# OllieBoyne/sslap

Hardware: AMD Instinct MI355X
Metric: Medges/s (bid-phase CSR nnz/s) + solve ms, N=200k d=0.1% sparse LAP (higher is better)
Workload: dtype f64

## Files before the change

### sslap_amd/csrc/device_common.hpp

```cpp
#pragma once
#include <hip/hip_runtime.h>
#include <stdint.h>

#include <type_traits>

namespace misslap {

constexpr int kWave = 64;
constexpr int kPosNone = 0x7fffffff;
constexpr int kTailMax = 512;

#define MISSLAP_KERNEL(BLOCK) MISSLAP_KERNEL_BOUND(BLOCK, BLOCK)
#define MISSLAP_KERNEL_BOUND(BLOCK, BOUND)                                                          \
    static constexpr int kBlock = (BLOCK);    \
    static constexpr int kBound = (BOUND);      \
    static_assert(kBlock <= kBound, "a launch above the kernel's bound fails");                     \
    template <class... A_>                                                                          \
    static __global__ __launch_bounds__(BOUND) void entry(A_... a_) {                               \
        run(a_...);                                                                                 \
    }

constexpr int kErrNegativeBid = 1;
constexpr int kErrRowsUnsorted = 2;
constexpr int kErrRowGap = 4;
// ... 105 lines not shown
}

__device__ __forceinline__ bool dense_entry_valid(double v) {
    const unsigned long long b = (unsigned long long)__double_as_longlong(v);
    return b <= 0x7ff0000000000000ull || b == 0x8000000000000000ull;
}
__device__ __forceinline__ bool bid_is_bad(double bid) {
    const unsigned long long b = (unsigned long long)__double_as_longlong(bid);
    return b > 0x7ff0000000000000ull;
}

__device__ __forceinline__ double shfl_xor_f64(double v, int off) {
    int lo = __double2loint(v), hi = __double2hiint(v);
    lo = __shfl_xor(lo, off);
    hi = __shfl_xor(hi, off);
    return __hiloint2double(hi, lo);
}

struct NoStamp {
    __device__ __forceinline__ void operator()(int) const {}
    __device__ __forceinline__ void light(int) const {}
};
struct CycleStamp {
    unsigned long long *acc;
    unsigned long long *prev;
    bool on;
    __device__ __forceinline__ void operator()(int k) const {
        asm volatile("s_waitcnt vmcnt(0) lgkmcnt(0)" ::: "memory");
        const unsigned long long t = __builtin_amdgcn_s_memtime();
        if (on) acc[k] += t - *prev;
        *prev = t;
    }
    __device__ __forceinline__ void light(int k) const {
        const unsigned long long t = __builtin_amdgcn_s_memtime();
        if (on) acc[k] += t - *prev;
        *prev = t;
    }
};

constexpr int kDppXor1 = 0xB1;
constexpr int kDppXor2 = 0x4E;
constexpr int kDppHalfMirror = 0x141;
constexpr int kDppMirror = 0x140;
constexpr int kDppBcast15 = 0x142;
constexpr int kDppBcast31 = 0x143;
template <int CTRL, int ROW_MASK = 0xF>
__device__ __forceinline__ int dpp_i32(int v) {
    return __builtin_amdgcn_update_dpp(v, v, CTRL, ROW_MASK, 0xF, false);
}
template <int CTRL, int ROW_MASK = 0xF>
__device__ __forceinline__ double dpp_f64(double v) {
    const int lo = dpp_i32<CTRL, ROW_MASK>(__double2loint(v));
    const int hi = dpp_i32<CTRL, ROW_MASK>(__double2hiint(v));
    return __hiloint2double(hi, lo);
}
__device__ __forceinline__ double readlane_f64(double v, int l) {
    const int lo = __builtin_amdgcn_readlane(__double2loint(v), l);
    const int hi = __builtin_amdgcn_readlane(__double2hiint(v), l);
    return __hiloint2double(hi, lo);
}

#define MISSLAP_WAVE_MAX_STEP(T, EXCH) \
    {                                  \
        const T o = EXCH;              \
        v = o > v ? o : v;             \
    }
__device__ __forceinline__ int wave_max_i32(int v) {
    MISSLAP_WAVE_MAX_STEP(int, __builtin_amdgcn_mov_dpp(v, kDppXor1, 0xF, 0xF, true))
    MISSLAP_WAVE_MAX_STEP(int, __builtin_amdgcn_mov_dpp(v, kDppXor2, 0xF, 0xF, true))
    MISSLAP_WAVE_MAX_STEP(int, __builtin_amdgcn_mov_dpp(v, kDppHalfMirror, 0xF, 0xF, true))
    MISSLAP_WAVE_MAX_STEP(int, __builtin_amdgcn_mov_dpp(v, kDppMirror, 0xF, 0xF, true))
    MISSLAP_WAVE_MAX_STEP(int, (dpp_i32<kDppBcast15, 0xA>(v)))
    MISSLAP_WAVE_MAX_STEP(int, (dpp_i32<kDppBcast31, 0xC>(v)))
    return __builtin_amdgcn_readlane(v, 63);
}
__device__ __forceinline__ double wave_max_f64(double v) {
    v = __builtin_fmax(v, dpp_f64<kDppXor1>(v));
    v = __builtin_fmax(v, dpp_f64<kDppXor2>(v));
    v = __builtin_fmax(v, dpp_f64<kDppHalfMirror>(v));
    v = __builtin_fmax(v, dpp_f64<kDppMirror>(v));
    v = __builtin_fmax(v, (dpp_f64<kDppBcast15, 0xA>(v)));
    v = __builtin_fmax(v, (dpp_f64<kDppBcast31, 0xC>(v)));
    return readlane_f64(v, 63);
}
#undef MISSLAP_WAVE_MAX_STEP

struct Top2 {
    double v, w;
    int g;
};
__device__ __forceinline__ Top2 top2_wave_reduce(const Top2 &x) {
    Top2 r;
    r.v = wave_max_f64(x.v);
    r.g = wave_max_i32(x.v == r.v ? x.g : -1);
    r.w = wave_max_f64(x.g == r.g ? x.w : x.v);
    return r;
}

struct __attribute__((aligned(16))) PriceRec {
    double price;
    int owner;
    int ostart;
};

__device__ __forceinline__ int lane_id() { return threadIdx.x & (kWave - 1); }
__device__ __forceinline__ unsigned long long lanemask_lt() {
    return (1ull << lane_id()) - 1ull;
}

constexpr int kCandLanes = 32;
constexpr int kCandMax = 30;
constexpr int kCandMin = 24;
constexpr int kCandRowMax = 4 * kWave;

template <int CTRL>
__device__ __forceinline__ int dppf_i32(int v) {
    return __builtin_amdgcn_mov_dpp(v, CTRL, 0xF, 0xF, true);
}
template <int CTRL>
__device__ __forceinline__ double dppf_f64(double v) {
    return __hiloint2double(dppf_i32<CTRL>(__double2hiint(v)), dppf_i32<CTRL>(__double2loint(v)));
}
__device__ __forceinline__ double half_max_f64(double v) {
    v = __builtin_fmax(v, dppf_f64<kDppXor1>(v));
    v = __builtin_fmax(v, dppf_f64<kDppXor2>(v));
    v = __builtin_fmax(v, dppf_f64<kDppHalfMirror>(v));
    v = __builtin_fmax(v, dppf_f64<kDppMirror>(v));
    v = __builtin_fmax(v, (dpp_f64<kDppBcast15, 0xA>(v)));
    return v;
}
__device__ __forceinline__ int half_max_i32(int v) {
    v = max(v, dppf_i32<kDppXor1>(v));
    v = max(v, dppf_i32<kDppXor2>(v));
    v = max(v, dppf_i32<kDppHalfMirror>(v));
    v = max(v, dppf_i32<kDppMirror>(v));
    v = max(v, (dpp_i32<kDppBcast15, 0xA>(v)));
    return v;
}
__device__ __forceinline__ int half_allmax_i32(int v) {
    v = max(v, dppf_i32<kDppXor1>(v));
    v = max(v, dppf_i32<kDppXor2>(v));
    v = max(v, dppf_i32<kDppHalfMirror>(v));
    v = max(v, dppf_i32<kDppMirror>(v));
    const auto s = __builtin_amdgcn_permlane16_swap(v, v, false, false);
    return max((int)s[0], (int)s[1]);
}

__device__ __forceinline__ double slot_cost(const int2 &s) { return (double)__int_as_float(s.y); }
__device__ __forceinline__ double slot_cost(const Slot64 &s) { return s.c; }
__device__ __forceinline__ double slot_cost_at(const int2 &s, int sl) {
    return (double)__int_as_float(__builtin_amdgcn_readlane(s.y, sl));
}
__device__ __forceinline__ double slot_cost_at(const Slot64 &s, int sl) { return readlane_f64(s.c, sl); }
template <class Slot>
struct LineIO;
template <>
struct LineIO<int2> {
    static __device__ __forceinline__ int2 load(const int2 *cand, const double *, size_t idx) { return cand[idx]; }
    static __device__ __forceinline__ int2 make(int x, int y) { return make_int2(x, y); }
};
template <>
struct LineIO<Slot64> {
    static __device__ __forceinline__ Slot64 load(const int2 *cand, const double *cost, size_t idx) {
        const int2 s = cand[idx];
        Slot64 r;
        r.x = s.x;
        r.y = s.y;
        r.c = cost[idx];
        return r;
    }
    static __device__ __forceinline__ Slot64 make(int x, int y) {
        Slot64 r;
        r.x = x;
        r.y = y;
        r.c = 0.0;
        return r;
    }
};

struct CandBid {
    bool hit;
    unsigned long long key;
    int obj;
    int prev, pstart;
    int len;
};

struct RecSource {
    const PriceRec *rec;
    __device__ __forceinline__ PriceRec get(int col) const { return rec[col]; }
};
struct PriceSource {
    const double *price;
    __device__ __forceinline__ PriceRec get(int col) const {
        PriceRec r;
        r.price = price[col];
        r.owner = -1;
        r.ostart = 0;
        return r;
    }
};

template <class Slot, class Src>
__device__ __forceinline__ PriceRec cand_gather2(const Slot slot, const bool act0, const bool act1, const Src &src) {
    const int lane = lane_id(), l32 = lane & (kCandLanes - 1);
    const bool active = lane < kCandLanes ? act0 : act1;
    const bool is_cand = active & (l32 >= 1) & (l32 <= kCandMax) & (slot.x >= 0);
    return src.get(is_cand ? slot.x : 0);
}
template <class Slot, class Early, class S = NoStamp>
__device__ __forceinline__ void cand_eval2_r(Slot &slot, const PriceRec r, const bool act0, const bool act1,
                                             const double eps, CandBid (&out)[2], int &err, Early &&early,
                                             const S &stamp = S(), int *alive = nullptr);
template <class Slot, class Src, class Early, class S = NoStamp>
__device__ __forceinline__ void cand_eval2(Slot &slot, const bool act0, const bool act1, const Src &src,
                                           const double eps, CandBid (&out)[2], int &err, Early &&early,
                                           const S &stamp = S(), int *alive = nullptr) {
    stamp(1);
    const PriceRec r = cand_gather2(slot, act0, act1, src);
    stamp(2);
    cand_eval2_r(slot, r, act0, act1, eps, out, err, early, stamp, alive);
}
template <class Slot, class Early, class S>
__device__ __forceinline__ void cand_eval2_r(Slot &slot, const PriceRec r, const bool act0, const bool act1,
                                             const double eps, CandBid (&out)[2], int &err, Early &&early,
                                             const S &stamp, int *alive) {
    const int lane = lane_id(), l32 = lane & (kCandLanes - 1);
    const double ninf = -__builtin_huge_val();
    const bool active = lane < kCandLanes ? act0 : act1;
    const bool is_cand = active & (l32 >= 1) & (l32 <= kCandMax) & (slot.x >= 0);
    const double cost = slot_cost(slot);
    double tau[2];
    tau[0] = readlane_f64(__hiloint2double(slot.y, slot.x), 0);
    tau[1] = readlane_f64(__hiloint2double(slot.y, slot.x), kCandLanes);
    out[0].len = __builtin_amdgcn_readlane(slot.x, kCandLanes - 1);
    out[1].len = __builtin_amdgcn_readlane(slot.x, 2 * kCandLanes - 1);
    const double v = is_cand ? cost - r.price : ninf;
    if (alive) {
        const unsigned long long al = __ballot(is_cand & (v >= (lane < kCandLanes ? tau[0] : tau[1])));
        alive[0] = __popc((unsigned)al);
        alive[1] = __popc((unsigned)(al >> 32));
    }
    double V[2], W[2];
    int G[2];
    {
        const double vm = half_max_f64(v);
        V[0] = readlane_f64(vm, 31);
        V[1] = readlane_f64(vm, 63);
        const double Vv = lane < kCandLanes ? V[0] : V[1];
        const int gm = half_max_i32((is_cand & (v == Vv)) ? l32 : -1);
        G[0] = __builtin_amdgcn_readlane(gm, 31);
        G[1] = __builtin_amdgcn_readlane(gm, 63);
    }
    double c1[2];
#pragma unroll
    for (int X = 0; X < 2; ++X) {
        const int sl = kCandLanes * X + max(G[X], 0);
        out[X].obj = __builtin_amdgcn_readlane(slot.x, sl);
        out[X].prev = __builtin_amdgcn_readlane(r.owner, sl);
        out[X].pstart = __builtin_amdgcn_readlane(r.ostart, sl);
        c1[X] = slot_cost_at(slot, sl);
    }
    early(out);
    stamp.light(3);
    const int Gv = lane < kCandLanes ? G[0] : G[1];
    const double wm = half_max_f64(l32 == Gv ? ninf : v);
    W[0] = readlane_f64(wm, 31);
    W[1] = readlane_f64(wm, 63);
#pragma unroll
    for (int X = 0; X < 2; ++X) {
        out[X].hit = (G[X] >= 0) & (V[X] > tau[X]) & (W[X] >= tau[X]);
        const double bid = (c1[X] - W[X]) + eps;
        if (out[X].hit && bid_is_bad(bid)) err |= kErrNegativeBid;
        out[X].key = bid_to_key(bid);
    }
}
template <class Slot, class Src>
__device__ __forceinline__ PriceRec cand_gather1(const Slot &slot, const bool cls, const Src &src) {
    const bool is_cand = cls & (slot.x >= 0);
    return src.get(is_cand ? slot.x : 0);
}
template <class Slot, class Early, class S = NoStamp>
__device__ __forceinline__ void cand_eval1_r(Slot &slot, const PriceRec r, const bool cls, const double eps, CandBid &out,
                                             unsigned &bad_hi, Early &&early, const S &stamp = S());
template <class Slot, class Src, class Early, class S = NoStamp>
__device__ __forceinline__ void cand_eval1(Slot &slot, const bool cls, const Src &src, const double eps, CandBid &out,
                                           unsigned &bad_hi, Early &&early, const S &stamp = S()) {
    stamp(1);
    const PriceRec r = cand_gather1(slot, cls, src);
    stamp(2);
    cand_eval1_r(slot, r, cls, eps, out, bad_hi, early, stamp);
}
template <class Slot, class Early, class S>
__device__ __forceinline__ void cand_eval1_r(Slot &slot, const PriceRec r, const bool cls, const double eps, CandBid &out,
                                             unsigned &bad_hi, Early &&early, const S &stamp) {
    const int lane = lane_id();
    const double ninf = -__builtin_huge_val();
    const bool is_cand = cls & (slot.x >= 0);
    const double cost = slot_cost(slot);
    const double tau = readlane_f64(__hiloint2double(slot.y, slot.x), 0);
    out.len = __builtin_amdgcn_readlane(slot.x, kCandLanes - 1);
    const double v = is_cand ? cost - r.price : ninf;
    const int hi = __double2hiint(v);
    const int k = hi ^ ((hi >> 31) & 0x7fffffff);
    const int km = __builtin_amdgcn_readlane(half_max_i32(k), 31);
    const unsigned eq = (unsigned)(__ballot(k == km) & 0xffffffffull);
    double V;
    int G;
    if (__popc(eq) == 1) {
        G = __ffs((int)eq) - 1;
        V = readlane_f64(v, G);
    } else {
        V = readlane_f64(half_max_f64(v), 31);
        G = __builtin_amdgcn_readlane(half_max_i32((is_cand & (v == V)) ? lane : -1), 31);
    }
    const int sl = max(G, 0);
    out.obj = __builtin_amdgcn_readlane(slot.x, sl);
    out.prev = __builtin_amdgcn_readlane(r.owner, sl);
    out.pstart = __builtin_amdgcn_readlane(r.ostart, sl);
    const double c1 = slot_cost_at(slot, sl);
    early(out);
    stamp.light(3);
    const double W = readlane_f64(half_max_f64(lane == G ? ninf : v), 31);
    out.hit = (G >= 0) & (V > tau) & (W >= tau);
    const double bid = (c1 - W) + eps;
    bad_hi = max(bad_hi, out.hit ? (unsigned)__double2hiint(bid) : 0u);
    out.key = bid_to_key(bid);
}
__device__ __forceinline__ bool bad_hi_is_error(unsigned bad_hi) { return bad_hi > 0x7ff00000u; }
struct NoEarly {
    __device__ __forceinline__ void operator()(const CandBid (&)[2]) const {}
    __device__ __forceinline__ void operator()(const CandBid &) const {}
};

struct CandBuildArgs {
    int c[4];
    double a[4], v[4];
    double V, W;
    int len;
    bool want;
};

__device__ __forceinline__ void cand_build(int2 *cand, double *cost, int person, const CandBuildArgs &ba, double eps,
// ... 266 lines not shown
```

### sslap_amd/csrc/kernels_tail.hpp

```cpp
#pragma once
#include "device_common.hpp"

namespace misslap {

struct TailArgs {
    Ctl *ctl;
    const int *row_ptr;
    double *price;
    PriceRec *rec;
    int *p2o;
    int *o2p;
    int *U;
    int2 *cand;
    double *cand64;
    int thr;
    int round_budget;
    float eps;
};

constexpr int kHashSize = 2048;

__device__ __forceinline__ unsigned long long readlane_u64(unsigned long long v, int l) {
    const int lo = __builtin_amdgcn_readlane((int)(unsigned)(v & 0xffffffffull), l);
    const int hi = __builtin_amdgcn_readlane((int)(unsigned)(v >> 32), l);
    return ((unsigned long long)(unsigned)hi << 32) | (unsigned long long)(unsigned)lo;
}

__device__ __forceinline__ int apply_winner(const TailArgs &a, int person, int pstart, int obj, int prev,
                                            unsigned long long key) {
    PriceRec r;
    r.price = key_to_bid(key);
    r.owner = person;
    r.ostart = pstart;
    a.rec[obj] = r;
    return prev;
}

struct k_sync_from_rec {
    MISSLAP_KERNEL(256)
    static __device__ __forceinline__ void run(Ctl *ctl, const PriceRec *rec, double *price, int *o2p, int *p2o, const int *U, int n_cols, int lines, unsigned long long *live, unsigned ticket) {
        const int K = ctl->K;
        if (blockIdx.x == 0 && threadIdx.x == 0) {
            post_live_status(live, ticket, K, ctl->err, ctl->nits);
            ctl->n_need = 0;
        }
        for (int n = blockIdx.x * blockDim.x + threadIdx.x; n < K; n += gridDim.x * blockDim.x) {
            const int i = U[n];
            if (i >= 0) p2o[i] = -1;
        }
        for (int j = blockIdx.x * blockDim.x + threadIdx.x; j < n_cols; j += gridDim.x * blockDim.x) {
            const PriceRec r = rec[j];
            if (lines && r.price < price[j]) atomicOr(&ctl->err, kErrPriceFell);
            price[j] = r.price;
            o2p[j] = r.owner;
            if (r.owner >= 0) p2o[r.owner] = j;
        }
    }
};


struct TailStats {
    unsigned long long edges, miss_edges, builds;
    unsigned bids, misses;
    unsigned bad_hi;
    int err;
    double hint;
};

__device__ __forceinline__ int lane_zero() {
    return (int)__builtin_amdgcn_mbcnt_hi(0u, __builtin_amdgcn_mbcnt_lo(0u, 0u));
}

template <class Slot>
__device__ __forceinline__ Slot cand_no_line() {
    return (lane_id() & (kCandLanes - 1)) == 0 ? LineIO<Slot>::make(0, 0x7ff00000) : LineIO<Slot>::make(-1, 0);
}
template <class E>
__device__ __forceinline__ typename E::Slot line_of(const TailArgs &a, int p, int l32) {
    return LineIO<typename E::Slot>::load(a.cand, a.cand64, (size_t)max(p, 0) * kCandLanes + l32);
}
template <class E>
struct TwoFetch {
    typename E::Slot slot;
    typename E::Raw row[2][4];
    int ev[2];
};
template <class E>
__device__ __forceinline__ void fetch_row(const TailArgs &a, const E &ed, int person, int start,
                                          typename E::Raw (&row)[4], int &e) {
    const int lane = lane_id();
#pragma unroll
    for (int u = 0; u < 4; ++u) row[u] = ed.load_raw_nt(start + u * kWave + lane);
    e = a.row_ptr[max(person, 0) + 1 + lane_zero()];
}
template <class E>
__device__ __forceinline__ void request_two(const TailArgs &a, const E &ed, int p0, int s0, int p1, int s1,
                                            TwoFetch<E> &tf) {
    if (E::kCand) {
        const int pme = lane_id() < kCandLanes ? p0 : p1;
        tf.slot = a.cand != nullptr ? line_of<E>(a, pme, lane_id() & (kCandLanes - 1)) : cand_no_line<typename E::Slot>();
    } else {
        fetch_row<E>(a, ed, p0, s0, tf.row[0], tf.ev[0]);
        fetch_row<E>(a, ed, p1, s1, tf.row[1], tf.ev[1]);
    }
}

__device__ __forceinline__ void tail_build(const TailArgs &a, int person, const CandBuildArgs &ba, double eps,
                                           TailStats &st) {
    cand_build(a.cand, a.cand64, person, ba, eps, st.hint);
    st.builds += 1;
}

template <class E, class Early, class S = NoStamp>
__device__ __forceinline__ void bid_two(const TailArgs &a, const E &ed, const int (&pi)[2], const int (&ps)[2],
                                        TwoFetch<E> &tf, double eps, CandBid (&b)[2], CandBuildArgs &bd,
                                        int &bd_person, TailStats &st, Early &&early, const S &stamp = S()) {
    const RecSource src{a.rec};
    b[0].hit = b[1].hit = false;
    if (E::kCand) cand_eval2(tf.slot, pi[0] >= 0, pi[1] >= 0, src, eps, b, st.err, early, stamp);
    stamp.light(4);
    bd_person = -1;
#pragma unroll
    for (int X = 0; X < 2; ++X) {
        if (pi[X] < 0) continue;
        if (!b[X].hit) {
            if (bd_person >= 0) tail_build(a, bd_person, bd, eps, st);
            if (E::kCand) {
                const typename E::Raw none[4] = {};
                const int e = a.row_ptr[pi[X] + 1 + lane_zero()];
                wave_bid_full<E, RecSource, true, false>(ed, src, ps[X], e, none, eps, b[X], bd, st.err);
            } else {
                wave_bid_full<E, RecSource, true, true>(ed, src, ps[X], tf.ev[X], tf.row[X], eps, b[X], bd, st.err);
            }
            bd.want = bd.want && a.cand != nullptr;
            bd_person = bd.want ? pi[X] : -1;
            st.misses += 1;
            st.miss_edges += (unsigned long long)b[X].len;
        }
        st.edges += (unsigned long long)b[X].len;
        st.bids += 1;
    }
}

__device__ __forceinline__ int round_limit(long long nits, long long max_iter) {
    return (int)min(max_iter - nits, (long long)0x7fffffff);
}

template <class E>
__device__ __forceinline__ void tail_chain_mode(const TailArgs &a, const E &ed, int &pi, int &ps, int &K,
                                                long long &nits, const long long max_iter, const double eps,
                                                TailStats &st) {
    const int lane = lane_id(), l32 = lane & (kCandLanes - 1);
    const RecSource src{a.rec};
    const bool cls = (lane >= 1) & (lane <= kCandMax);
    const bool lines = E::kCand && a.cand != nullptr;
    typename E::Slot slot = cand_no_line<typename E::Slot>();
    typename E::Raw row[4];
    int ev = 0;
    auto request = [&](int person, int start) {
        if (E::kCand) {
            if (lines) slot = line_of<E>(a, person, l32);
        } else {
            fetch_row<E>(a, ed, person, start, row, ev);
        }
    };
    request(pi, ps);
    const int rmax = round_limit(nits, max_iter);
    int r = 0;
#ifdef MISSLAP_TAIL_STAMP
    unsigned long long sacc[8] = {0, 0, 0, 0, 0, 0, 0, 0}, sprev = __builtin_amdgcn_s_memtime();
    const CycleStamp stamp{sacc, &sprev, true};
#else
    const NoStamp stamp;
#endif
    for (;;) {
        CandBid b;
        b.hit = false;
        int sp = -2;
        if (E::kCand)
            cand_eval1(slot, cls, src, eps, b, st.bad_hi, [&](const CandBid &w) {
                sp = w.prev;
                request(sp, 0);
            }, stamp);
        stamp.light(4);
        if (!b.hit) {
            CandBuildArgs bd;
            if (E::kCand) {
                const typename E::Raw none[4] = {};
                const int e = a.row_ptr[pi + 1];
                wave_bid_full<E, RecSource, true, false>(ed, src, ps, e, none, eps, b, bd, st.err);
            } else {
                wave_bid_full<E, RecSource, true, true>(ed, src, ps, ev, row, eps, b, bd, st.err);
            }
            st.misses += 1;
            st.miss_edges += (unsigned long long)b.len;
            if (bd.want && lines) tail_build(a, pi, bd, eps, st);
        }
        stamp.light(5);
        st.edges += (unsigned long long)b.len;
        st.bids += 1;
        r += 1;
        if (lane == 0) apply_winner(a, pi, ps, b.obj, b.prev, b.key);
        pi = b.prev;
        ps = b.pstart;
        const bool done = pi < 0 || r >= rmax;
        if (!done && sp != pi) request(pi, ps);
        stamp.light(6);
        if (done) break;
    }
    K = pi != -1;
    nits += r;
#ifdef MISSLAP_TAIL_STAMP
    if (lane == 0) {
        for (int k = 1; k <= 6; ++k) a.ctl->dbg[5 + k] += sacc[k];
    }
#endif
}

template <class E>
__device__ __forceinline__ void tail_solo_mode(const TailArgs &a, const E &ed, int *sU, int *sStart, int &K,
                                               long long &nits, const long long max_iter, const double eps,
                                               TailStats &st) {
    const int lane = lane_id();
    int pi[2], ps[2];
    pi[0] = __builtin_amdgcn_readfirstlane(sU[0]);
    ps[0] = __builtin_amdgcn_readfirstlane(sStart[0]);
    pi[1] = K > 1 ? __builtin_amdgcn_readfirstlane(sU[1]) : -1;
    ps[1] = K > 1 ? __builtin_amdgcn_readfirstlane(sStart[1]) : 0;
    if (K == 1) {
        tail_chain_mode(a, ed, pi[0], ps[0], K, nits, max_iter, eps, st);
        if (lane == 0) {
            sU[0] = pi[0];
            sU[1] = -1;
            sStart[0] = ps[0];
        }
        return;
    }
    TwoFetch<E> tf;
    tf.slot = cand_no_line<typename E::Slot>();
    request_two(a, ed, pi[0], ps[0], pi[1], ps[1], tf);
#ifdef MISSLAP_TAIL_STAMP_SOLO
    unsigned long long sacc[8] = {0, 0, 0, 0, 0, 0, 0, 0}, sprev = __builtin_amdgcn_s_memtime();
    const CycleStamp stamp{sacc, &sprev, true};
#else
    const NoStamp stamp;
#endif
    for (;;) {
        CandBid b[2];
        CandBuildArgs bd;
        int bd_person;
        int sp[2] = {-2, -2};
        bid_two(a, ed, pi, ps, tf, eps, b, bd, bd_person, st, [&](const CandBid(&w)[2]) {
            sp[0] = pi[0] >= 0 ? w[0].prev : -1;
            sp[1] = pi[1] >= 0 ? w[1].prev : -1;
            request_two(a, ed, sp[0], 0, sp[1], 0, tf);
        }, stamp);
        stamp.light(5);
        nits += 1;
        bool win0 = true, win1 = pi[1] >= 0;
        if (win1 && b[0].obj == b[1].obj) {
            if (b[1].key > b[0].key) win0 = false;
            else win1 = false;
        }
        if (lane == 0) {
            if (win0) apply_winner(a, pi[0], ps[0], b[0].obj, b[0].prev, b[0].key);
            if (win1) apply_winner(a, pi[1], ps[1], b[1].obj, b[1].prev, b[1].key);
        }
        if (win0) {
            pi[0] = b[0].prev;
            ps[0] = b[0].pstart;
        }
        if (win1) {
            pi[1] = b[1].prev;
            ps[1] = b[1].pstart;
        }
        if (pi[0] == -1 && pi[1] != -1) {
            pi[0] = pi[1];
            ps[0] = ps[1];
            pi[1] = -1;
        }
        K = (pi[0] != -1) + (pi[1] != -1);
        const bool done = K <= 1 || nits >= max_iter;
        if (!done && (sp[0] != pi[0] || sp[1] != pi[1])) request_two(a, ed, pi[0], ps[0], pi[1], ps[1], tf);
        if (bd_person >= 0) tail_build(a, bd_person, bd, eps, st);
        stamp.light(6);
        if (done) break;
    }
    if (K == 1 && nits < max_iter) tail_chain_mode(a, ed, pi[0], ps[0], K, nits, max_iter, eps, st);
#ifdef MISSLAP_TAIL_STAMP_SOLO
    if (lane == 0)
        for (int k = 1; k <= 6; ++k) a.ctl->dbg[5 + k] += sacc[k];
#endif
    if (lane == 0) {
        sU[0] = pi[0];
        sU[1] = pi[1];
        sStart[0] = ps[0];
        sStart[1] = ps[1];
    }
}

template <class E>
__device__ __forceinline__ void tail_pair_mode(const TailArgs &a, const E &ed, int *sU, int *sStart, int &K,
                                               long long &nits, const long long max_iter, const double eps,
                                               TailStats &st) {
    const int lane = lane_id(), l32 = lane & (kCandLanes - 1);
    const bool upper = lane >= kCandLanes;
    const RecSource src{a.rec};
    const bool cls = (l32 >= 1) & (l32 <= kCandMax);
    const double ninf = -__builtin_huge_val();
    int pi[2], ps[2];
#pragma unroll
    for (int X = 0; X < 2; ++X) {
        pi[X] = __builtin_amdgcn_readfirstlane(sU[X]);
        ps[X] = __builtin_amdgcn_readfirstlane(sStart[X]);
    }
    typename E::Slot slot;
    auto request = [&](int p0, int p1) { slot = line_of<E>(a, upper ? p1 : p0, l32); };
    const int rmax = round_limit(nits, max_iter);
    int r = 0;
    if (K == 2) request(pi[0], pi[1]);
#ifdef MISSLAP_TAIL_STAMP_DUO
    unsigned long long sacc[8] = {0, 0, 0, 0, 0, 0, 0, 0}, sprev = __builtin_amdgcn_s_memtime();
    const CycleStamp stamp{sacc, &sprev, true};
#else
    const NoStamp stamp;
#endif
    while (K == 2) {
        stamp(1);
        const PriceRec g = cand_gather1(slot, cls, src);
        stamp(2);
        const bool is_cand = cls & (slot.x >= 0);
        const double v = is_cand ? slot_cost(slot) - g.price : ninf;
        const int hw = __double2hiint(v);
        const int k = hw ^ ((hw >> 31) & 0x7fffffff);
        const unsigned long long eq = __ballot(k == half_allmax_i32(k));
        const unsigned eq0 = (unsigned)eq, eq1 = (unsigned)(eq >> 32);
        int G[2];
        double V[2];
        if ((int)(__popc(eq0) == 1) & (int)(__popc(eq1) == 1)) {
            G[0] = __ffs((int)eq0) - 1;
            G[1] = __ffs((int)eq1) + (kCandLanes - 1);
            V[0] = readlane_f64(v, G[0]);
            V[1] = readlane_f64(v, G[1]);
        } else {
            const double vm = half_max_f64(v);
            V[0] = readlane_f64(vm, kCandLanes - 1);
            V[1] = readlane_f64(vm, kWave - 1);
            const int gm = half_max_i32((is_cand & (v == (upper ? V[1] : V[0]))) ? lane : -1);
            G[0] = __builtin_amdgcn_readlane(gm, kCandLanes - 1);
            G[1] = __builtin_amdgcn_readlane(gm, kWave - 1);
        }
        CandBid b[2];
        double tau[2], c1[2];
#pragma unroll
        for (int X = 0; X < 2; ++X) {
            const int sl = max(G[X], kCandLanes * X);
            tau[X] = readlane_f64(__hiloint2double(slot.y, slot.x), kCandLanes * X);
            b[X].len = __builtin_amdgcn_readlane(slot.x, kCandLanes * X + kCandLanes - 1);
            b[X].obj = __builtin_amdgcn_readlane(slot.x, sl);
            b[X].prev = __builtin_amdgcn_readlane(g.owner, sl);
            b[X].pstart = __builtin_amdgcn_readlane(g.ostart, sl);
            c1[X] = slot_cost_at(slot, sl);
        }
        const int sp0 = b[0].prev, sp1 = b[1].prev;
        request(sp0, sp1);
        stamp.light(3);
        const double wm = half_max_f64(((lane == G[0]) | (lane == G[1])) ? ninf : v);
        const double W[2] = {readlane_f64(wm, kCandLanes - 1), readlane_f64(wm, kWave - 1)};
#pragma unroll
        for (int X = 0; X < 2; ++X) {
            b[X].hit = (G[X] >= 0) & (V[X] > tau[X]) & (W[X] >= tau[X]);
            const double bid = (c1[X] - W[X]) + eps;
            st.bad_hi = max(st.bad_hi, b[X].hit ? (unsigned)__double2hiint(bid) : 0u);
            b[X].key = bid_to_key(bid);
        }
        stamp.light(4);
#pragma unroll
        for (int X = 0; X < 2; ++X) {
            if (!b[X].hit) {
                CandBuildArgs bd;
                const typename E::Raw none[4] = {};
                const int e = a.row_ptr[pi[X] + 1];
                wave_bid_full<E, RecSource, true, false>(ed, src, ps[X], e, none, eps, b[X], bd, st.err);
                st.misses += 1;
                st.miss_edges += (unsigned long long)b[X].len;
                if (bd.want) tail_build(a, pi[X], bd, eps, st);
            }
        }
        stamp.light(5);
        st.edges += (unsigned long long)(b[0].len + b[1].len);
        st.bids += 2;
        r += 1;
        if ((b[0].obj != b[1].obj) & (b[0].prev >= 0) & (b[1].prev >= 0)) {
            if (l32 == 0) {
                PriceRec w;
                w.price = key_to_bid(upper ? b[1].key : b[0].key);
                w.owner = upper ? pi[1] : pi[0];
                w.ostart = upper ? ps[1] : ps[0];
                a.rec[upper ? b[1].obj : b[0].obj] = w;
            }
#pragma unroll
            for (int X = 0; X < 2; ++X) {
                pi[X] = b[X].prev;
                ps[X] = b[X].pstart;
            }
        } else {
            bool win0 = true, win1 = true;
            if (b[0].obj == b[1].obj) {
                if (b[1].key > b[0].key) win0 = false;
                else win1 = false;
            }
            if (lane == 0) {
                if (win0) apply_winner(a, pi[0], ps[0], b[0].obj, b[0].prev, b[0].key);
                if (win1) apply_winner(a, pi[1], ps[1], b[1].obj, b[1].prev, b[1].key);
            }
            if (win0) {
                pi[0] = b[0].prev;
                ps[0] = b[0].pstart;
            }
            if (win1) {
                pi[1] = b[1].prev;
                ps[1] = b[1].pstart;
            }
            if (pi[0] == -1 && pi[1] != -1) {
                pi[0] = pi[1];
                ps[0] = ps[1];
                pi[1] = -1;
            }
            K = (pi[0] != -1) + (pi[1] != -1);
        }
        const bool done = K <= 1 || r >= rmax;
        if (!done && (sp0 != pi[0] || sp1 != pi[1])) request(pi[0], pi[1]);
        stamp.light(6);
        if (done) break;
    }
    nits += r;
#ifdef MISSLAP_TAIL_STAMP_DUO
    if (lane == 0)
        for (int k = 1; k <= 6; ++k) a.ctl->dbg[5 + k] += sacc[k];
#endif
    if (K == 1 && nits < max_iter) tail_chain_mode(a, ed, pi[0], ps[0], K, nits, max_iter, eps, st);
    if (lane == 0) {
        sU[0] = pi[0];
        sU[1] = pi[1];
        sStart[0] = ps[0];
        sStart[1] = ps[1];
    }
}

constexpr int kTeamMax = 16;
constexpr int kTeamTab = 64;
__device__ __forceinline__ void tail_barrier_lds() { asm volatile("s_waitcnt lgkmcnt(0)\n\ts_barrier" ::: "memory"); }

template <class E>
__device__ __forceinline__ void tail_team_mode(const TailArgs &a, const E &ed, int *sU, int *sStart, int &K,
                                               long long &nits, const long long max_iter, const double eps,
                                               TailStats &st) {
    const int lane = lane_id(), wave = __builtin_amdgcn_readfirstlane(threadIdx.x >> 6);
    static_assert(kTeamMax <= 2 * (kTailMax / kWave) && kTeamMax <= kWave, "two list slots per wavefront");
    __shared__ unsigned long long tKey[2][kTeamMax];
    __shared__ int tObj[2][kTeamMax], tPrev[2][kTeamMax], tPst[2][kTeamMax], tU[2][kTeamMax], tS[2][kTeamMax];
    __shared__ int wTab[kTailMax / kWave][kTeamTab];
    const int n0 = 2 * wave;
    int pi[2], ps[2];
#pragma unroll
    for (int X = 0; X < 2; ++X) {
        pi[X] = n0 + X < K ? __builtin_amdgcn_readfirstlane(sU[min(n0 + X, kTailMax - 1)]) : -1;
        ps[X] = n0 + X < K ? __builtin_amdgcn_readfirstlane(sStart[min(n0 + X, kTailMax - 1)]) : 0;
    }
    wTab[wave][lane & (kTeamTab - 1)] = -1;
    TwoFetch<E> tf;
    tf.slot = cand_no_line<typename E::Slot>();
    if (n0 < K) request_two(a, ed, pi[0], ps[0], pi[1], ps[1], tf);
    __syncthreads();
#ifdef MISSLAP_TAIL_STAMP_TEAM
    unsigned long long sacc[8] = {0, 0, 0, 0, 0, 0, 0, 0}, sprev = __builtin_amdgcn_s_memtime();
    const CycleStamp stamp{sacc, &sprev, wave == 0};
#else
    const NoStamp stamp;
#endif
    int par = 0;
    for (;;) {
        int sp[2] = {-2, -2};
        CandBuildArgs bd;
        int bd_person = -1;
        stamp.light(0);
        if (n0 < K) {
            CandBid b[2];
            bid_two(a, ed, pi, ps, tf, eps, b, bd, bd_person, st, [&](const CandBid(&w)[2]) {
                sp[0] = pi[0] >= 0 ? w[0].prev : -1;
                sp[1] = pi[1] >= 0 ? w[1].prev : -1;
                request_two(a, ed, sp[0], 0, sp[1], 0, tf);
            });
            if (lane == 0) {
#pragma unroll
                for (int X = 0; X < 2; ++X)
                    if (pi[X] >= 0) {
                        tKey[par][n0 + X] = b[X].key;
                        tObj[par][n0 + X] = b[X].obj;
                        tPrev[par][n0 + X] = b[X].prev;
                        tPst[par][n0 + X] = b[X].pstart;
                        tU[par][n0 + X] = pi[X];
                        tS[par][n0 + X] = ps[X];
                    }
            }
        }
        stamp.light(1);
        tail_barrier_lds();
        stamp.light(2);
        {
            const bool act = lane < K;
            const int ls = min(lane, kTeamMax - 1);
            const unsigned long long lkey = act ? tKey[par][ls] : 0ull;
            const int lobj = act ? tObj[par][ls] : (-2 - lane);
            const int lprev = act ? tPrev[par][ls] : 0, lpst = act ? tPst[par][ls] : 0;
            int u = act ? tU[par][ls] : -1;
            int sx = act ? tS[par][ls] : 0;
            int hs = 0;
            bool dup = false;
            if (act) {
                hs = (int)(((unsigned)lobj * 2654435761u) >> 26) & (kTeamTab - 1);
                for (;;) {
                    const int old = atomicCAS(&wTab[wave][hs], -1, lobj);
                    if (old == -1) break;
                    if (old == lobj) {
                        dup = true;
                        break;
                    }
                    hs = (hs + 1) & (kTeamTab - 1);
                }
            }
            const bool contested = __any(dup);
            if (act && !dup) wTab[wave][hs] = -1;
            const bool ends = __any(act && lprev == -1);
#ifdef MISSLAP_TAIL_STAMP_TEAM
            if (threadIdx.x == 0) sacc[5] += (!contested && !ends), sacc[6] += contested, sacc[7] += 1;
#endif
            if (!contested && !ends) {
                if (act && n0 < K) apply_winner(a, u, sx, lobj, lprev, lkey);
#pragma unroll
                for (int X = 0; X < 2; ++X) {
                    const int w = __builtin_amdgcn_readlane(lprev, min(n0 + X, kWave - 1));
                    const int ws = __builtin_amdgcn_readlane(lpst, min(n0 + X, kWave - 1));
                    pi[X] = n0 + X < K ? w : -1;
                    ps[X] = n0 + X < K ? ws : 0;
                }
            } else {
                bool lose = false;
                for (int m = 0; m < K; ++m) {
                    const int om = __builtin_amdgcn_readlane(lobj, m);
                    const bool same = (om == lobj) && (m != lane);
                    if (__any(same)) {
                        const unsigned long long km = readlane_u64(lkey, m);
                        lose |= same && (km > lkey || (km == lkey && m < lane));
                    }
                }
                const bool won = act && !lose;
                if (won && n0 < K) apply_winner(a, u, sx, lobj, lprev, lkey);
                u = won ? lprev : u;
                sx = won ? lpst : sx;
                const unsigned long long kmask = (1ull << K) - 1ull;
                const unsigned long long holes = __ballot(act && u == -1) & kmask;
                const int Kn = K - __popcll(holes);
                const unsigned long long lmask = (1ull << Kn) - 1ull;
                unsigned long long hl = holes & lmask;
                unsigned long long mv = ~holes & ~lmask & kmask;
                while (hl) {
                    const int hk = __ffsll((long long)hl) - 1, mk = __ffsll((long long)mv) - 1;
                    const int mu = __builtin_amdgcn_readlane(u, mk), ms = __builtin_amdgcn_readlane(sx, mk);
                    if (lane == hk) {
                        u = mu;
                        sx = ms;
                    }
                    hl &= hl - 1;
                    mv &= mv - 1;
                }
                K = Kn;
#pragma unroll
                for (int X = 0; X < 2; ++X) {
                    pi[X] = n0 + X < K ? __builtin_amdgcn_readlane(u, min(n0 + X, kWave - 1)) : -1;
                    ps[X] = n0 + X < K ? __builtin_amdgcn_readlane(sx, min(n0 + X, kWave - 1)) : 0;
                }
            }
        }
        stamp.light(3);
        par ^= 1;
        nits += 1;
        const bool done = K <= 2 || nits >= max_iter;
        if (!done && n0 < K && (sp[0] != pi[0] || sp[1] != pi[1]))
            request_two(a, ed, pi[0], ps[0], pi[1], ps[1], tf);
        if (bd_person >= 0) tail_build(a, bd_person, bd, eps, st);
        stamp.light(4);
        if (done) break;
    }
#ifdef MISSLAP_TAIL_STAMP_TEAM
    if (threadIdx.x == 0)
        for (int k = 1; k <= 6; ++k) a.ctl->dbg[5 + k] += sacc[k];
#endif
    if (lane < 2 && n0 + lane < kTeamMax) {
        sU[n0 + lane] = lane == 0 ? pi[0] : pi[1];
        sStart[n0 + lane] = lane == 0 ? ps[0] : ps[1];
    }
    __syncthreads();
}

constexpr int kPipeTab = 4096;
__device__ __forceinline__ int pipe_hash(int obj) { return (int)(((unsigned)obj * 2654435761u) >> 20); }
static_assert((1 << 12) == kPipeTab, "pipe_hash keeps the top 12 bits");
struct __attribute__((aligned(16))) PipeSlot {
    PriceRec rec;
    int4 aux;
};
struct __attribute__((aligned(16))) PipeLds {
    PipeSlot slot[2][kTeamMax];
    int dirty[2];
    int pad[2];
    int tab[kPipeTab];
};

__device__ __forceinline__ void touch_slot(const int2 &s) { asm volatile("" ::"v"(s.x), "v"(s.y)); }
__device__ __forceinline__ void touch_slot(const Slot64 &s) { asm volatile("" ::"v"(s.x), "v"(s.y), "v"(s.c)); }

template <class E>
__device__ __forceinline__ bool tail_team1_pipe(const TailArgs &a, const E &ed, int *sU, int *sStart, int &K,
                                                long long &nits, const long long max_iter, const double eps,
                                                TailStats &st) {
    const int lane = lane_id(), l32 = lane & (kCandLanes - 1);
    const int wave = __builtin_amdgcn_readfirstlane(threadIdx.x >> 6);
    __shared__ PipeLds L;
    const RecSource src{a.rec};
    const bool cls = (lane >= 1) & (lane <= kCandMax);
    const int n0 = wave;
    int pi = n0 < K ? __builtin_amdgcn_readfirstlane(sU[min(n0, kTailMax - 1)]) : -1;
    int ps = n0 < K ? __builtin_amdgcn_readfirstlane(sStart[min(n0, kTailMax - 1)]) : 0;
    for (int h = threadIdx.x; h < kPipeTab; h += blockDim.x) L.tab[h] = -1;
    if (threadIdx.x < 2) L.dirty[threadIdx.x] = -1;
    typename E::Slot slot = cand_no_line<typename E::Slot>();
    auto request = [&](int person) { slot = line_of<E>(a, person, l32); };
    if (n0 < K) request(pi);
    __syncthreads();
#ifdef MISSLAP_TAIL_STAMP_TEAM
    unsigned long long sacc[8] = {0, 0, 0, 0, 0, 0, 0, 0}, sprev = __builtin_amdgcn_s_memtime();
    const CycleStamp stamp{sacc, &sprev, wave == 0};
#else
    const NoStamp stamp;
#endif
    const int rmax = round_limit(nits, max_iter);
    int r = 0;
    int par = 0;
    const int ls = min(lane, kTeamMax - 1);
    PriceRec grec = PriceRec{0.0, -1, 0};
    bool have_g = false;
    for (;;) {
        if (n0 >= K) {
            if (lane == 0) {
                sU[n0] = -1;
                sStart[n0] = 0;
            }
            tail_barrier_lds();
            nits += r;
            return true;
        }
        int sp = -2;
        CandBid b;
        b.hit = false;
        stamp.light(0);
        if (!have_g) grec = cand_gather1(slot, cls, src);
#ifdef MISSLAP_TAIL_STAMP_TEAM
        asm volatile("s_waitcnt vmcnt(0)" ::: "memory");
        stamp.light(1);
#endif
        cand_eval1_r(slot, grec, cls, eps, b, st.bad_hi, [&](const CandBid &w) {
            sp = w.prev;
            request(sp);
        });
        if (!b.hit) {
            CandBuildArgs bd;
            const typename E::Raw none[4] = {};
            const int e = a.row_ptr[pi + 1 + lane_zero()];
            wave_bid_full<E, RecSource, true, false>(ed, src, ps, e, none, eps, b, bd, st.err);
            st.misses += 1;
            st.miss_edges += (unsigned long long)b.len;
            if (bd.want) tail_build(a, pi, bd, eps, st);
        }
        st.edges += (unsigned long long)b.len;
        st.bids += 1;
        stamp.light(2);
        if (lane == 0) {
            const int old = atomicExch(&L.tab[pipe_hash(b.obj)], r);
            PriceRec mine;
            mine.price = key_to_bid(b.key);
            mine.owner = pi;
            mine.ostart = ps;
            L.slot[par][n0].rec = mine;
            L.slot[par][n0].aux = make_int4(b.obj, b.prev, b.pstart, 0);
            if (old == r || b.prev < 0) L.dirty[par] = r;
        }
        stamp.light(3);
        tail_barrier_lds();
        stamp.light(4);
        {
            const int dflag = L.dirty[par];
            const PriceRec lrec = L.slot[par][ls].rec;
            const int lobj = L.slot[par][ls].aux.x;
#ifdef MISSLAP_TAIL_STAMP_TEAM
            asm volatile("s_waitcnt lgkmcnt(0)" ::: "memory");
            stamp.light(5);
#endif
            if (__builtin_amdgcn_readfirstlane(dflag) != r) {
                have_g = sp == b.prev;
                if (have_g) {
                    touch_slot(slot);
                    if (lane < K) a.rec[lobj] = lrec;
                    grec = cand_gather1(slot, cls, src);
                } else {
                    if (lane < K) a.rec[lobj] = lrec;
                }
                pi = b.prev;
                ps = b.pstart;
            } else {
                have_g = false;
                const bool act = lane < K;
                const int4 laux = L.slot[par][ls].aux;
                const unsigned long long lkey = act ? bid_to_key(lrec.price) : 0ull;
                const int lo = act ? laux.x : (-2 - lane);
                const int lprev = act ? laux.y : 0, lpst = act ? laux.z : 0;
                int u = act ? lrec.owner : -1;
                int sx = act ? lrec.ostart : 0;
                bool lose = false;
                for (int m = 0; m < K; ++m) {
                    const int om = __builtin_amdgcn_readlane(lo, m);
                    const bool same = (om == lo) && (m != lane);
                    if (__any(same)) {
                        const unsigned long long km = readlane_u64(lkey, m);
                        lose |= same && (km > lkey || (km == lkey && m < lane));
                    }
                }
                const bool won = act && !lose;
                if (won) apply_winner(a, u, sx, lo, lprev, lkey);
                u = won ? lprev : u;
                sx = won ? lpst : sx;
                const unsigned long long kmask = (1ull << K) - 1ull;
                const unsigned long long holes = __ballot(act && u == -1) & kmask;
                const int Kn = K - __popcll(holes);
                const unsigned long long lmask = (1ull << Kn) - 1ull;
                unsigned long long hl = holes & lmask;
                unsigned long long mv = ~holes & ~lmask & kmask;
                while (hl) {
                    const int hk = __ffsll((long long)hl) - 1, mk = __ffsll((long long)mv) - 1;
                    const int mu = __builtin_amdgcn_readlane(u, mk), ms = __builtin_amdgcn_readlane(sx, mk);
                    if (lane == hk) {
                        u = mu;
                        sx = ms;
                    }
                    hl &= hl - 1;
                    mv &= mv - 1;
                }
                K = Kn;
                pi = n0 < K ? __builtin_amdgcn_readlane(u, min(n0, kWave - 1)) : -1;
                ps = n0 < K ? __builtin_amdgcn_readlane(sx, min(n0, kWave - 1)) : 0;
            }
        }
        par ^= 1;
        r += 1;
        const bool done = K <= 2 || r >= rmax;
        if (!done && n0 < K && sp != pi) request(pi);
        stamp.light(6);
        if (done) break;
    }
    nits += r;
#ifdef MISSLAP_TAIL_STAMP_TEAM
    if (threadIdx.x == 0)
        for (int k = 1; k <= 6; ++k) a.ctl->dbg[5 + k] += sacc[k];
#endif
    if (lane == 0 && n0 < kTeamMax) {
        sU[n0] = pi;
        sStart[n0] = ps;
    }
    __syncthreads();
    return false;
}

template <class E, int kThreads, bool kTeamOnly = false>
struct k_tail {
    MISSLAP_KERNEL(kThreads)
    static __device__ __forceinline__ void run(TailArgs a, E ed) {
        static_assert(!kTeamOnly || (kThreads == 2 * kTailMax && kThreads / kWave == kTeamMax), "one slot per wavefront");
        constexpr bool kBlockOnly = kThreads > kTailMax && !kTeamOnly;
        constexpr bool kDuoOnly = kThreads == kWave;
        static_assert(!kDuoOnly || !kTeamOnly, "roles are exclusive");
        __shared__ int sU[kTailMax];
        __shared__ unsigned long long sKey[kTailMax];
        __shared__ int sObj[kTailMax];
        __shared__ int sPrev[kTailMax];
        __shared__ int sStart[kTailMax];
        __shared__ int sPst[kTailMax];
        __shared__ int sList[kTailMax];
        __shared__ int hObj[kHashSize];
        __shared__ unsigned long long hKey[kHashSize];
        __shared__ int hPos[kHashSize];
        __shared__ int sCnt[3][kThreads / kWave];
        __shared__ int sK, sMissCnt;
        __shared__ long long sNits;

        Ctl *ctl = a.ctl;
        const int t = threadIdx.x, lane = t & 63, wave = t >> 6;
        constexpr int nwaves = kThreads / kWave;
        int K = ctl->K;
        long long nits = ctl->nits;
        const long long max_iter =
            a.round_budget > 0 ? min(ctl->max_iter, nits + (long long)(kBlockOnly ? max(a.round_budget / 4, 1) : a.round_budget))
                               : ctl->max_iter;
        if (K == 0 || K > a.thr || nits >= max_iter) return;
        if (kBlockOnly && K <= kTeamMax) return;
        if (kTeamOnly && (K <= 2 || K > kTeamMax)) return;
        if (kDuoOnly && (K > 2 || !E::kCand || a.cand == nullptr)) return;
        if (!kBlockOnly && !kTeamOnly && a.round_budget > 0 && K > 2 && E::kCand && a.cand != nullptr) return;
        const int K0 = K;
        const long long nits0 = nits;
        for (int n = t; n < kTailMax; n += kThreads) {
            sU[n] = (n < K) ? a.U[n] : -1;
            sStart[n] = (n < K) ? a.row_ptr[sU[n]] : 0;
        }
        if (!kDuoOnly)
            for (int h = t; h < kHashSize; h += kThreads) {
                hObj[h] = -1;
                hKey[h] = 0ull;
                hPos[h] = kPosNone;
            }
        const double eps = (double)a.eps;
        TailStats st;
        st.edges = st.miss_edges = st.builds = 0ull;
        st.bids = st.misses = st.bad_hi = 0u;
        st.err = 0;
        st.hint = 0.0;
        if (t == 0) sMissCnt = 0;
        __syncthreads();

        unsigned long long md[6] = {0, 0, 0, 0, 0, 0};
#ifdef MISSLAP_TAIL_STAMP_BLOCK
        unsigned long long bacc[8] = {0, 0, 0, 0, 0, 0, 0, 0};
#endif
        auto mode_begin = [&](int m) {
            md[3 + m] -= __builtin_amdgcn_s_memrealtime();
            md[m] -= (unsigned long long)nits;
        };
        auto mode_end = [&](int m) {
            md[3 + m] += __builtin_amdgcn_s_memrealtime();
            md[m] += (unsigned long long)nits;
        };
        auto flush_stats = [&]() {
            if (lane == 0) {
                if (st.bids) {
                    const unsigned long long hits = (unsigned long long)(st.bids - st.misses), hit_edges = st.edges - st.miss_edges;
                    atomicAdd(&ctl->edges, st.edges);
                    atomicAdd(&ctl->tail_edges, st.edges);
                    atomicAdd(&ctl->bids, (unsigned long long)st.bids);
                    if (hits) {
                        atomicAdd(&ctl->cand_hits, hits);
                        atomicAdd(&ctl->cand_edges, hit_edges);
                    }
                    atomicAdd(&ctl->dbg[12], (unsigned long long)st.bids);
                    atomicAdd(&ctl->dbg[13], hits);
                    atomicAdd(&ctl->dbg[14], st.builds);
                    atomicAdd(&ctl->dbg[15], hit_edges);
                }
                if (bad_hi_is_error(st.bad_hi)) st.err |= kErrNegativeBid;
                if (st.err) atomicOr(&ctl->err, st.err);
            }
        };
        for (;;) {
            if (kBlockOnly && K <= kTeamMax) break;
            if (kDuoOnly) {
                mode_begin(0);
                tail_pair_mode(a, ed, sU, sStart, K, nits, max_iter, eps, st);
                mode_end(0);
                break;
            }
            if (kTeamOnly) {
                if (K > 2 && nits < max_iter) {
                    mode_begin(1);
                    if (tail_team1_pipe(a, ed, sU, sStart, K, nits, max_iter, eps, st)) {
                        flush_stats();
                        return;
                    }
                    mode_end(1);
                }
                break;
            }
            if (!kBlockOnly && K <= 2) {
                if (wave == 0) {
                    mode_begin(0);
                    tail_solo_mode(a, ed, sU, sStart, K, nits, max_iter, eps, st);
                    mode_end(0);
                    if (lane == 0) {
                        sK = K;
                        sNits = nits;
                    }
                }
                __syncthreads();
                K = sK;
                nits = sNits;
                break;
            }
            if (!kBlockOnly && K <= kTeamMax) {
                mode_begin(1);
                tail_team_mode(a, ed, sU, sStart, K, nits, max_iter, eps, st);
                mode_end(1);
                if (K == 0 || nits >= max_iter) break;
                continue;
            }
            mode_begin(2);
#ifdef MISSLAP_TAIL_STAMP_BLOCK
            unsigned long long sprev_b = __builtin_amdgcn_s_memtime();
            const CycleStamp bstamp{bacc, &sprev_b, wave == 0};
#else
            const NoStamp bstamp;
#endif
            {
                const RecSource src{a.rec};
                constexpr int kBlockDepth = kBlockOnly ? 1 : 3;
                for (int base = 0; base < K; base += kBlockDepth * 2 * nwaves) {
                    typename E::Slot sl[kBlockDepth];
                    PriceRec rr[kBlockDepth];
#pragma unroll
                    for (int c = 0; c < kBlockDepth; ++c) {
                        const int nme = base + c * 2 * nwaves + 2 * wave + (lane >> 5);
                        const int pme = nme < K ? sU[min(nme, kTailMax - 1)] : -1;
                        sl[c] = cand_no_line<typename E::Slot>();
                        if (E::kCand && a.cand != nullptr) sl[c] = line_of<E>(a, pme, lane & (kCandLanes - 1));
                    }
                    bstamp(1);
#pragma unroll
                    for (int c = 0; c < kBlockDepth; ++c) {
                        const int n0 = base + c * 2 * nwaves + 2 * wave;
                        if (E::kCand) rr[c] = cand_gather2(sl[c], n0 < K, n0 + 1 < K, src);
                    }
                    bstamp(2);
#pragma unroll
                    for (int c = 0; c < kBlockDepth; ++c) {
                        const int n0 = base + c * 2 * nwaves + 2 * wave;
                        if (n0 >= K) continue;
                        CandBid b[2];
                        b[0].hit = b[1].hit = false;
                        if (E::kCand) cand_eval2_r(sl[c], rr[c], n0 < K, n0 + 1 < K, eps, b, st.err, NoEarly());
#pragma unroll
                        for (int X = 0; X < 2; ++X) {
                            const int n = n0 + X;
                            if (n >= K) continue;
                            if (b[X].hit) {
                                if (lane == 0) {
                                    sKey[n] = b[X].key;
                                    sObj[n] = b[X].obj;
                                    sPrev[n] = b[X].prev;
                                    sPst[n] = b[X].pstart;
                                }
                                st.edges += (unsigned long long)b[X].len;
                                st.bids += 1;
                            } else if (lane == 0) {
                                sList[atomicAdd(&sMissCnt, 1)] = n;
                            }
                        }
                    }
                }
                __syncthreads();
// ... 200 lines not shown
```

Measured before the change: 4811.

## Use explicit global-address-space loads/stores and explicit vmem waits in tail chain/duo loops

Tail chain and duo loops now load candidate lines, price records and row pointers through address_space(1) pointers so the compiler emits global rather than flat memory instructions. The winner record is stored by all lanes as one 16-byte vector store instead of a lane-0 apply_winner. Explicit s_waitcnt vmcnt drains are added after requests, and readfirstlane is applied to the round limit and K to keep them scalar. The aim is lower per-round latency in the latency-bound serial tail. The risk is that removing apply_winner's side effects (such as o2p/p2o updates) or the multi-lane store changes semantics, and the forced waits could reduce overlap.

```diff
diff --git a/sslap_amd/csrc/device_common.hpp b/sslap_amd/csrc/device_common.hpp
--- a/sslap_amd/csrc/device_common.hpp
+++ b/sslap_amd/csrc/device_common.hpp
@@ -281,11 +281,35 @@
     return (double)__int_as_float(__builtin_amdgcn_readlane(s.y, sl));
 }
 __device__ __forceinline__ double slot_cost_at(const Slot64 &s, int sl) { return readlane_f64(s.c, sl); }
+#define MISSLAP_GLOBAL __attribute__((address_space(1)))
+typedef int GlobalInt2 __attribute__((ext_vector_type(2), may_alias));
+typedef int GlobalInt4 __attribute__((ext_vector_type(4), may_alias));
+__device__ __forceinline__ PriceRec rec_load_global(const PriceRec *p) {
+    const GlobalInt4 v = *(const MISSLAP_GLOBAL GlobalInt4 *)p;
+    PriceRec r;
+    r.price = __hiloint2double(v.y, v.x);
+    r.owner = v.z;
+    r.ostart = v.w;
+    return r;
+}
+__device__ __forceinline__ void rec_store_global(PriceRec *p, const PriceRec &r) {
+    GlobalInt4 v;
+    v.x = __double2loint(r.price);
+    v.y = __double2hiint(r.price);
+    v.z = r.owner;
+    v.w = r.ostart;
+    *(MISSLAP_GLOBAL GlobalInt4 *)p = v;
+}
+
 template <class Slot>
 struct LineIO;
 template <>
 struct LineIO<int2> {
     static __device__ __forceinline__ int2 load(const int2 *cand, const double *, size_t idx) { return cand[idx]; }
+    static __device__ __forceinline__ int2 load_global(const int2 *cand, const double *, size_t idx) {
+        const GlobalInt2 s = *(const MISSLAP_GLOBAL GlobalInt2 *)(cand + idx);
+        return make_int2(s.x, s.y);
+    }
     static __device__ __forceinline__ int2 make(int x, int y) { return make_int2(x, y); }
 };
 template <>
@@ -298,6 +322,14 @@
         r.c = cost[idx];
         return r;
     }
+    static __device__ __forceinline__ Slot64 load_global(const int2 *cand, const double *cost, size_t idx) {
+        const GlobalInt2 s = *(const MISSLAP_GLOBAL GlobalInt2 *)(cand + idx);
+        Slot64 r;
+        r.x = s.x;
+        r.y = s.y;
+        r.c = *(const MISSLAP_GLOBAL double *)(cost + idx);
+        return r;
+    }
     static __device__ __forceinline__ Slot64 make(int x, int y) {
         Slot64 r;
         r.x = x;
@@ -318,6 +350,10 @@
 struct RecSource {
     const PriceRec *rec;
     __device__ __forceinline__ PriceRec get(int col) const { return rec[col]; }
+};
+struct RecSourceGlobal {
+    const PriceRec *rec;
+    __device__ __forceinline__ PriceRec get(int col) const { return rec_load_global(rec + col); }
 };
 struct PriceSource {
     const double *price;
diff --git a/sslap_amd/csrc/kernels_tail.hpp b/sslap_amd/csrc/kernels_tail.hpp
--- a/sslap_amd/csrc/kernels_tail.hpp
+++ b/sslap_amd/csrc/kernels_tail.hpp
@@ -80,6 +80,10 @@
     return LineIO<typename E::Slot>::load(a.cand, a.cand64, (size_t)max(p, 0) * kCandLanes + l32);
 }
 template <class E>
+__device__ __forceinline__ typename E::Slot line_of_global(const TailArgs &a, int p, int l32) {
+    return LineIO<typename E::Slot>::load_global(a.cand, a.cand64, (size_t)max(p, 0) * kCandLanes + l32);
+}
+template <class E>
 struct TwoFetch {
     typename E::Slot slot;
     typename E::Raw row[2][4];
@@ -142,8 +146,25 @@
     }
 }
 
+__device__ __forceinline__ void touch_slot(const int2 &s) { asm volatile("" ::"v"(s.x), "v"(s.y)); }
+__device__ __forceinline__ void touch_slot(const Slot64 &s) { asm volatile("" ::"v"(s.x), "v"(s.y), "v"(s.c)); }
+
+__device__ __forceinline__ void vmem_drained() { __builtin_amdgcn_s_waitcnt(0x0070); }
+
+template <class Slot>
+__device__ __forceinline__ void round_head_stamp(const NoStamp &, const Slot &) {}
+template <class Slot>
+__device__ __forceinline__ void round_head_stamp(const CycleStamp &stamp, const Slot &slot) {
+#ifdef MISSLAP_TAIL_STAMP_ACK
+    stamp(1);
+#else
+    touch_slot(slot);
+    stamp.light(1);
+#endif
+}
+
 __device__ __forceinline__ int round_limit(long long nits, long long max_iter) {
-    return (int)min(max_iter - nits, (long long)0x7fffffff);
+    return __builtin_amdgcn_readfirstlane((int)min(max_iter - nits, (long long)0x7fffffff));
 }
 
 template <class E>
@@ -159,12 +180,13 @@
     int ev = 0;
     auto request = [&](int person, int start) {
         if (E::kCand) {
-            if (lines) slot = line_of<E>(a, person, l32);
+            if (lines) slot = line_of_global<E>(a, person, l32);
         } else {
             fetch_row<E>(a, ed, person, start, row, ev);
         }
     };
     request(pi, ps);
+    vmem_drained();
     const int rmax = round_limit(nits, max_iter);
     int r = 0;
 #ifdef MISSLAP_TAIL_STAMP
@@ -177,17 +199,21 @@
         CandBid b;
         b.hit = false;
         int sp = -2;
-        if (E::kCand)
-            cand_eval1(slot, cls, src, eps, b, st.bad_hi, [&](const CandBid &w) {
+        if (E::kCand) {
+            round_head_stamp(stamp, slot);
+            const PriceRec g = cand_gather1(slot, cls, RecSourceGlobal{a.rec});
+            stamp(2);
+            cand_eval1_r(slot, g, cls, eps, b, st.bad_hi, [&](const CandBid &w) {
                 sp = w.prev;
                 request(sp, 0);
             }, stamp);
+        }
         stamp.light(4);
         if (!b.hit) {
             CandBuildArgs bd;
             if (E::kCand) {
                 const typename E::Raw none[4] = {};
-                const int e = a.row_ptr[pi + 1];
+                const int e = *(const MISSLAP_GLOBAL int *)(a.row_ptr + pi + 1);
                 wave_bid_full<E, RecSource, true, false>(ed, src, ps, e, none, eps, b, bd, st.err);
             } else {
                 wave_bid_full<E, RecSource, true, true>(ed, src, ps, ev, row, eps, b, bd, st.err);
@@ -195,16 +221,26 @@
             st.misses += 1;
             st.miss_edges += (unsigned long long)b.len;
             if (bd.want && lines) tail_build(a, pi, bd, eps, st);
+            vmem_drained();
         }
         stamp.light(5);
         st.edges += (unsigned long long)b.len;
         st.bids += 1;
         r += 1;
-        if (lane == 0) apply_winner(a, pi, ps, b.obj, b.prev, b.key);
+        {
+            PriceRec w;
+            w.price = key_to_bid(b.key);
+            w.owner = pi;
+            w.ostart = ps;
+            rec_store_global(&a.rec[b.obj], w);
+        }
         pi = b.prev;
         ps = b.pstart;
         const bool done = pi < 0 || r >= rmax;
-        if (!done && sp != pi) request(pi, ps);
+        if (!done && sp != pi) {
+            request(pi, ps);
+            vmem_drained();
+        }
         stamp.light(6);
         if (done) break;
     }
@@ -315,10 +351,11 @@
         ps[X] = __builtin_amdgcn_readfirstlane(sStart[X]);
     }
     typename E::Slot slot;
-    auto request = [&](int p0, int p1) { slot = line_of<E>(a, upper ? p1 : p0, l32); };
+    auto request = [&](int p0, int p1) { slot = line_of_global<E>(a, upper ? p1 : p0, l32); };
     const int rmax = round_limit(nits, max_iter);
     int r = 0;
     if (K == 2) request(pi[0], pi[1]);
+    vmem_drained();
 #ifdef MISSLAP_TAIL_STAMP_DUO
     unsigned long long sacc[8] = {0, 0, 0, 0, 0, 0, 0, 0}, sprev = __builtin_amdgcn_s_memtime();
     const CycleStamp stamp{sacc, &sprev, true};
@@ -326,8 +363,8 @@
     const NoStamp stamp;
 #endif
     while (K == 2) {
-        stamp(1);
-        const PriceRec g = cand_gather1(slot, cls, src);
+        round_head_stamp(stamp, slot);
+        const PriceRec g = cand_gather1(slot, cls, RecSourceGlobal{a.rec});
         stamp(2);
         const bool is_cand = cls & (slot.x >= 0);
         const double v = is_cand ? slot_cost(slot) - g.price : ninf;
@@ -380,25 +417,27 @@
             if (!b[X].hit) {
                 CandBuildArgs bd;
                 const typename E::Raw none[4] = {};
-                const int e = a.row_ptr[pi[X] + 1];
+                const int e = *(const MISSLAP_GLOBAL int *)(a.row_ptr + pi[X] + 1);
                 wave_bid_full<E, RecSource, true, false>(ed, src, ps[X], e, none, eps, b[X], bd, st.err);
                 st.misses += 1;
                 st.miss_edges += (unsigned long long)b[X].len;
                 if (bd.want) tail_build(a, pi[X], bd, eps, st);
+                vmem_drained();
             }
         }
         stamp.light(5);
         st.edges += (unsigned long long)(b[0].len + b[1].len);
         st.bids += 2;
         r += 1;
+        {
+            const bool second = b[0].obj == b[1].obj ? b[1].key > b[0].key : upper;
+            PriceRec w;
+            w.price = key_to_bid(second ? b[1].key : b[0].key);
+            w.owner = second ? pi[1] : pi[0];
+            w.ostart = second ? ps[1] : ps[0];
+            rec_store_global(&a.rec[upper ? b[1].obj : b[0].obj], w);
+        }
         if ((b[0].obj != b[1].obj) & (b[0].prev >= 0) & (b[1].prev >= 0)) {
-            if (l32 == 0) {
-                PriceRec w;
-                w.price = key_to_bid(upper ? b[1].key : b[0].key);
-                w.owner = upper ? pi[1] : pi[0];
-                w.ostart = upper ? ps[1] : ps[0];
-                a.rec[upper ? b[1].obj : b[0].obj] = w;
-            }
 #pragma unroll
             for (int X = 0; X < 2; ++X) {
                 pi[X] = b[X].prev;
@@ -410,10 +449,6 @@
                 if (b[1].key > b[0].key) win0 = false;
                 else win1 = false;
             }
-            if (lane == 0) {
-                if (win0) apply_winner(a, pi[0], ps[0], b[0].obj, b[0].prev, b[0].key);
-                if (win1) apply_winner(a, pi[1], ps[1], b[1].obj, b[1].prev, b[1].key);
-            }
             if (win0) {
                 pi[0] = b[0].prev;
                 ps[0] = b[0].pstart;
@@ -430,7 +465,10 @@
             K = (pi[0] != -1) + (pi[1] != -1);
         }
         const bool done = K <= 1 || r >= rmax;
-        if (!done && (sp0 != pi[0] || sp1 != pi[1])) request(pi[0], pi[1]);
+        if (!done && (sp0 != pi[0] || sp1 != pi[1])) {
+            request(pi[0], pi[1]);
+            vmem_drained();
+        }
         stamp.light(6);
         if (done) break;
     }
@@ -617,9 +655,6 @@
     int pad[2];
     int tab[kPipeTab];
 };
-
-__device__ __forceinline__ void touch_slot(const int2 &s) { asm volatile("" ::"v"(s.x), "v"(s.y)); }
-__device__ __forceinline__ void touch_slot(const Slot64 &s) { asm volatile("" ::"v"(s.x), "v"(s.y), "v"(s.c)); }
 
 template <class E>
 __device__ __forceinline__ bool tail_team1_pipe(const TailArgs &a, const E &ed, int *sU, int *sStart, int &K,
@@ -811,6 +846,7 @@
         const long long max_iter =
             a.round_budget > 0 ? min(ctl->max_iter, nits + (long long)(kBlockOnly ? max(a.round_budget / 4, 1) : a.round_budget))
                                : ctl->max_iter;
+        if (kDuoOnly) K = __builtin_amdgcn_readfirstlane(K);
         if (K == 0 || K > a.thr || nits >= max_iter) return;
         if (kBlockOnly && K <= kTeamMax) return;
         if (kTeamOnly && (K <= 2 || K > kTeamMax)) return;
```

Result: no change. 4804 (-0.1%).
